# zyang1580/PDA

Measured on AMD Instinct MI355X. Metric: users/sec full-catalogue top-K@50 (eval), higher is better.
Workload: dtype f32; 1 GPU; C3: synthetic 1000000 users x 200000 items, d=128, PDA condition ((elu+1)*pop^0.22) head, masked top-K@50; ranks_seen=1

## Files before the change

pda_amd/csrc/pda_score_topk_v4.hip:

```cpp
#include "pda_v4_shared.h"
#include <cstdlib>
#include <type_traits>

using namespace pda_topk;

namespace {

constexpr int kCap4 = 57;
constexpr int kRing4 = 128;
constexpr int kWarmTiles = 4;
constexpr int kMainWaves = 8;
#ifndef PDA_W4_ABL
#define PDA_W4_ABL 0
#endif
#ifdef PDA_V4_PROF
__device__ unsigned long long pda_prof4[24];
#define PROF_T0(v) const long long v = __builtin_readcyclecounter()
#define PROF_T1(v, slot) prof[slot] += (unsigned long long)(__builtin_readcyclecounter() - v)
#define PROF_INC(slot, x) prof[slot] += (unsigned long long)(x)
#define PROF_FLUSH(first, last) do { if (lane == 0) for (int pq = (first); pq <= (last); ++pq) atomicAdd(&pda_prof4[pq], prof[pq]); } while (0)
#else
#define PROF_T0(v) do {} while (0)
#define PROF_T1(v, slot) do {} while (0)
#define PROF_INC(slot, x) do {} while (0)
// ... 560 lines not shown
    const int cap_t = (g.warm_sorted || g.handover != nullptr || g.warm_final) ? CAP : K;
    auto emit_row = [&](const int r, const uint32_t t, const int c_t) __attribute__((always_inline)) {
        const int row = (r & 3) + 8 * (r >> 2) + 4 * h;
        const int lrow = wave * 32 + row;
        if (j == 0) predt[lrow] = c_t >= K ? pda_unordf(t) : -INFINITY;
        if (__any(c_t > cap_t)) {
#pragma unroll
            for (int k = 0; k < NHT; ++k) {
                const bool p = ordv[k][r] >= t;
                const uint64_t key = ((uint64_t)ordv[k][r] << 32) | (uint64_t)(0xFFFFFFFFu - (uint32_t)itemv[k]);
                append_keys<CAP>(p, lrow, pda_unordf(ordv[k][r]), key, lists, cntl, taul, wave * 32, 32, K, lane);
            }
        } else {
            int run = 0;
#pragma unroll
            for (int k = 0; k < NHT; ++k) {
                const bool p = ordv[k][r] >= t;
                const uint64_t bm = __ballot(p);
                const uint32_t bh = h ? (uint32_t)(bm >> 32) : (uint32_t)bm;
                const int slot = run + __popc(bh & ((1u << j) - 1u));
                if (p) lists[(size_t)lrow * CAP + slot] = ((uint64_t)ordv[k][r] << 32) | (uint64_t)(0xFFFFFFFFu - (uint32_t)itemv[k]);
                run += __popc(bh);
            }
            if (j == 0) cntl[lrow] = run;
        }
    };
#pragma unroll
    for (int r = 0; r < 16; r += 2) {
        if constexpr ((PDA_W4_ABL & 2) != 0) {
#if defined(__HIP_DEVICE_COMPILE__)
#pragma unroll
            for (int k = 0; k < NHT; ++k) asm volatile("" ::"v"(ordv[k][r]), "v"(ordv[k][r + 1]));
#endif
            continue;
        }
        auto count_ge2 = [&](uint32_t ca, uint32_t cb, int& na, int& nb) __attribute__((always_inline)) {
            int loa = 0, hia = 0, lob = 0, hib = 0;
#pragma unroll
            for (int k = 0; k < NHT; ++k) {
                const uint64_t bma = __ballot(ordv[k][r] >= ca);
                const uint64_t bmb = __ballot(ordv[k][r + 1] >= cb);
                loa += __popc((uint32_t)bma);
                hia += __popc((uint32_t)(bma >> 32));
                lob += __popc((uint32_t)bmb);
                hib += __popc((uint32_t)(bmb >> 32));
            }
            na = h ? hia : loa;
            nb = h ? hib : lob;
        };
        int ca_t, cb_t;
        count_ge2(1u, 1u, ca_t, cb_t);
        uint32_t ta = 1u, tb = 1u;
        const bool needa = ca_t > cap_t, needb = cb_t > cap_t;
        if (__any(needa || needb)) {
            uint32_t mxa = 0u, mna = 0xFFFFFFFFu, mxb = 0u, mnb = 0xFFFFFFFFu;
#pragma unroll
            for (int k = 0; k < NHT; ++k) {
                const uint32_t va = ordv[k][r], vb = ordv[k][r + 1];
                mxa = max(mxa, va);
                mna = min(mna, va != 0u ? va : 0xFFFFFFFFu);
                mxb = max(mxb, vb);
                mnb = min(mnb, vb != 0u ? vb : 0xFFFFFFFFu);
            }
#pragma unroll
            for (int o = 16; o >= 1; o >>= 1) {
                mxa = max(mxa, (uint32_t)__shfl_xor((int)mxa, o, 64));
                mna = min(mna, (uint32_t)__shfl_xor((int)mna, o, 64));
                mxb = max(mxb, (uint32_t)__shfl_xor((int)mxb, o, 64));
                mnb = min(mnb, (uint32_t)__shfl_xor((int)mnb, o, 64));
            }
            uint32_t hia = mxa + 1u, hib = mxb + 1u;
            if (needa) ta = mna;
            if (needb) tb = mnb;
            for (int it = 0; it < 40; ++it) {
                const bool opena = needa && ca_t > cap_t && hia - ta > 1u;
                const bool openb = needb && cb_t > cap_t && hib - tb > 1u;
                if (!__any(opena || openb)) break;
                const uint32_t mida = opena ? ta + ((hia - ta) >> 1) : ta;
                const uint32_t midb = openb ? tb + ((hib - tb) >> 1) : tb;
                int cnta, cntb;
                count_ge2(mida, midb, cnta, cntb);
                if (opena) {
                    if (cnta >= K) {
                        ta = mida;
                        ca_t = cnta;
                    } else {
                        hia = mida;
                    }
                }
                if (openb) {
                    if (cntb >= K) {
                        tb = midb;
                        cb_t = cntb;
                    } else {
                        hib = midb;
                    }
                }
            }
        }
        emit_row(r, ta, ca_t);
        emit_row(r + 1, tb, cb_t);
    }
    pda_wave_sync();
    if (tid == 0) atomicAdd(reinterpret_cast<unsigned long long*>(g.stats + 2), (unsigned long long)(2 * nwarm));
    for (int rr = 0; rr < 32; ++rr) {
        uint64_t* buf = my_lists + rr * CAP;
        if (((PDA_W4_ABL & 4) == 0) && (g.warm_sorted || g.warm_final || (g.handover == nullptr && __builtin_amdgcn_readfirstlane(cntl[wave * 32 + rr]) > K)))
            compact_list<CAP>(buf, &cntl[wave * 32 + rr], &taul[wave * 32 + rr], K, lane);
        const int c = cntl[wave * 32 + rr];
        const int rb = utile * kUserTile + wave * 32 + rr;
        if (g.seed_out != nullptr) {
            uint32_t mn = lane < c ? (uint32_t)(buf[lane] >> 32) : 0xFFFFFFFFu;
#pragma unroll
            for (int o = 32; o >= 1; o >>= 1) mn = min(mn, (uint32_t)__shfl_xor((int)mn, o, 64));
            if (lane == 0 && rb < g.n_users_blk) g.seed_out[rb] = c >= K ? pda_unordf(mn) : -INFINITY;
        }
        if (g.kth_ws != nullptr) continue;
        if (g.handover != nullptr) {
            if (rb < g.n_users_blk && lane < CAP) g.handover[((size_t)split * g.n_users_blk + rb) * CAP + lane] = lane < c ? buf[lane] : 0ull;
            if (g.warm_final && rb < g.n_users_blk && lane < K) g.out_keys[((size_t)split * g.n_users_blk + rb) * K + lane] = lane < c ? buf[lane] : 0ull;
        } else if (rb < g.n_users_blk && lane < K) {
            const uint64_t k = lane < c ? buf[lane] : 0ull;
            g.out_keys[((size_t)split * g.n_users_blk + rb) * K + lane] = k;
        }
    }
    if (g.kth_ws != nullptr) {
        pda_wave_sync();
        const int rb0 = utile * kUserTile + wave * 32, nv = max(0, min(32, g.n_users_blk - rb0));
        if (lane < nv) {
            const uint64_t kl = my_lists[(size_t)lane * CAP + (K - 1)];
            g.kth_ws[(size_t)split * g.n_users_blk + rb0 + lane] = cntl[wave * 32 + lane] >= K ? pda_unordf((uint32_t)(kl >> 32)) : -INFINITY;
        }
        uint64_t* ob = g.out_keys + ((size_t)split * g.n_users_blk + rb0) * K;
        const int q64 = 64 / K, r64 = 64 % K;
        int rr = lane / K, p = lane % K;
        for (int i = lane; i < nv * K; i += 64) {
            ob[i] = p < cntl[wave * 32 + rr] ? my_lists[(size_t)rr * CAP + p] : 0ull;
            rr += q64;
            p += r64;
            if (p >= K) { p -= K; ++rr; }
        }
    }
    if (g.pred_ws != nullptr && lane < 32) {
        const int rb = utile * kUserTile + wave * 32 + lane;
        if (rb < g.n_users_blk) {
            g.pred_ws[2 * (size_t)rb] = predt[wave * 32 + lane];
            g.pred_ws[2 * (size_t)rb + 1] = nul[wave * 32 + lane];
        }
    }
}

constexpr int kWS5Waves = 8, kWS5Threads = 64 * kWS5Waves;
constexpr int kWarmPos = 64 * kWarmTiles;
constexpr size_t warm_score5_lds(int d) { return (size_t)kWarmPos * d * 4 + kWarmPos * 8 + (size_t)kWS5Waves * 32 * 2 * kWarmTiles * 4; }

template <int D, bool BF>
__global__ void __launch_bounds__(kWS5Threads) warm_score5_kernel(Args4 g) {
    extern __shared__ __attribute__((aligned(16))) unsigned char smem[];
    constexpr int RB = row_bytes(D);
    constexpr int NC = D / 8;
    constexpr int CPR4 = D / 4;
    float* Bt = reinterpret_cast<float*>(smem);
    float* popw = Bt + kWarmPos * D;
    int* idw = reinterpret_cast<int*>(popw + kWarmPos);
    unsigned* hmask = reinterpret_cast<unsigned*>(idw + kWarmPos);

    const int tid = threadIdx.x, lane = tid & 63, wave = tid >> 6;
    const int j = lane & 31, h = lane >> 5;
    const int nwarm = g.warm_tiles;
    const int npos = 64 * nwarm;
    for (int p = tid; p < npos; p += kWS5Threads) {
        const float* tl = reinterpret_cast<const float*>(g.rows + (size_t)p * RB + 2 * D + 32);
        popw[p] = tl[0];
        idw[p] = reinterpret_cast<const int*>(tl)[1];
    }
    __syncthreads();
    for (int id = tid; id < npos * CPR4; id += kWS5Threads) {
        const int jj = id / CPR4, ch = id % CPR4;
        *reinterpret_cast<f32x4*>(Bt + jj * D + 4 * (ch ^ swz<D>(jj & 31))) = pda_load4<BF>(g.I, (size_t)idw[jj] * D + 4 * ch);
    }
    if (blockIdx.x == 0) {
        for (int p = tid; p < kWarmPos; p += kWS5Threads) g.wscore[p] = p < npos ? (uint32_t)idw[p] : 0u;
        if (tid == 0) g.stats[8] = 5u;
    }
    __syncthreads();

    uint32_t* scores = g.wscore + kWarmPos;
    const int utiles_w = (g.n_users_blk + kUserTile - 1) / kUserTile;
    const int nunits = utiles_w * (kUserTile / 32);
    const int G = (int)gridDim.x, stride = G * kWS5Waves;
    unsigned* hm_l = hmask + wave * 32 * 2 * kWarmTiles;
    static_assert(2 * kWarmTiles == 8, "two 16-byte loads per row");

    auto row_uid = [&](int unit) -> int {
        const int rb = unit * 32 + j;
        return (unit < nunits && rb < g.n_users_blk) ? g.users[rb] : 0;
    };
    auto load_rows = [&](int unit_x, int uid, f32x4 (&a)[NC], u32x4& hm, bool& hm_on) __attribute__((always_inline)) {
        if (unit_x >= nunits) return;
        const int rb = unit_x * 32 + j;
#pragma unroll
        for (int c = 0; c < NC; ++c) a[c] = pda_load4<BF>(g.U, (size_t)uid * D + 4 * h + 8 * c);
        hm_on = false;
        if (g.hmask_tab != nullptr) {
            hm_on = rb < g.n_users_blk && (unsigned)uid < (unsigned)g.hmask_tab_rows;
            hm = *reinterpret_cast<const u32x4*>(g.hmask_tab + (size_t)(hm_on ? uid : 0) * (2 * kWarmTiles) + 4 * h);
        } else if (g.hmask_ws != nullptr) {
            hm_on = true;
            hm = *reinterpret_cast<const u32x4*>(g.hmask_ws + (size_t)rb * (2 * kWarmTiles) + 4 * h);
        }
    };
    unsigned long long n_tiles_done = 0ull;
    auto run_unit = [&](const int unit_in, f32x4 (&areg)[NC], const u32x4& hm_in, const bool hm_on) __attribute__((always_inline)) {
        const int unit = __builtin_amdgcn_readfirstlane(unit_in);
        const int row_blk = unit * 32 + j;
        if (unit * 32 + 32 > g.n_users_blk) {
            const f32x4 z = {0.f, 0.f, 0.f, 0.f};
#pragma unroll
            for (int c = 0; c < NC; ++c) areg[c] = row_blk < g.n_users_blk ? areg[c] : z;
        }
        const u32x4 hz = {0u, 0u, 0u, 0u};
        const u32x4 hmv = hm_on ? hm_in : hz;
        *reinterpret_cast<u32x4*>(hm_l + j * (2 * kWarmTiles) + 4 * h) = hmv;
        {
            constexpr int NK5 = D / 32;
            unsigned char* fb = g.ufrag_out + ((size_t)(row_blk >> 4) * (NK5 * 64) + (size_t)(row_blk & 15)) * 16 + 8 * h;
            float ssc[NC];
#pragma unroll
            for (int c = 0; c < NC; ++c) {
                const f32x4 v = areg[c];
                uint2 w;
                w.x = bf16_rne(v[0]) | (bf16_rne(v[1]) << 16);
                w.y = bf16_rne(v[2]) | (bf16_rne(v[3]) << 16);
                *reinterpret_cast<uint2*>(fb + ((c >> 2) * 64 + 16 * (c & 3)) * 16) = w;
                float ss = 0.f;
#pragma unroll
                for (int k = 0; k < 4; ++k) {
                    const float sq = v[k] * v[k];
                    ss += sq + __shfl_xor(sq, 32, 64);
                }
                ssc[c] = ss;
                __builtin_amdgcn_sched_barrier(0);
            }
#pragma unroll
            for (int o = NC / 2; o > 0; o >>= 1)
#pragma unroll
                for (int c = 0; c < o; ++c) ssc[c] += ssc[c + o];
            if (h == 0) g.unorm_out[row_blk] = sqrtf(ssc[0]) * 1.0009765625f * 1.0001f;
        }
        if ((unit & (kUserTile / 32 - 1)) == 0) n_tiles_done += (unsigned long long)(2 * nwarm);
        pda_wave_sync();
        const int j_lane = j, h_lane = h;
#pragma unroll 1
        for (int ht = 0; ht < 2 * nwarm; ++ht) {
            int j = j_lane, h = h_lane;
#if defined(__HIP_DEVICE_COMPILE__)
            asm volatile("" : "+v"(j), "+v"(h));
#endif
            const int bswz = swz<D>(j);
            const float* brow = Bt + (ht * 32 + j) * D;
            f32x16 acc0 = zero16v(), acc1 = zero16v();
            f32x4 b0 = *reinterpret_cast<const f32x4*>(brow + 4 * (h ^ bswz));
            f32x4 b1 = *reinterpret_cast<const f32x4*>(brow + 4 * ((2 + h) ^ bswz));
#pragma unroll
            for (int c = 0; c < NC; c += 2) {
                f32x4 n0 = b0, n1 = b1;
                if (c + 2 < NC) {
                    n0 = *reinterpret_cast<const f32x4*>(brow + 4 * ((2 * c + 4 + h) ^ bswz));
                    n1 = *reinterpret_cast<const f32x4*>(brow + 4 * ((2 * c + 6 + h) ^ bswz));
                }
#pragma unroll
                for (int q = 0; q < 4; ++q) {
                    acc0 = __builtin_amdgcn_mfma_f32_32x32x2f32(areg[c][q], b0[q], acc0, 0, 0, 0);
                    acc1 = __builtin_amdgcn_mfma_f32_32x32x2f32(areg[c + 1][q], b1[q], acc1, 0, 0, 0);
                }
                __builtin_amdgcn_sched_barrier(0);
                b0 = n0;
                b1 = n1;
            }
            const f32x16 accx = acc0 + acc1;
            const bool okw = (ht * 32 + j) < g.n_items_local;
            const float pv = popw[ht * 32 + j];
            const unsigned hb_mine = hm_l[j * (2 * kWarmTiles) + ht];
            const bool any_hb = __any(hb_mine != 0u);
            const uint32_t soff = (uint32_t)(unit * 32 + 4 * h) * (uint32_t)npos + (uint32_t)(ht * 32 + j);
#pragma unroll
            for (int r = 0; r < 16; ++r) {
                const int row = (r & 3) + 8 * (r >> 2) + 4 * h;
                float sc = accx[r];
                sc = (sc > 0.0f ? sc + 1.0f : __expf(sc)) * pv;
                bool p = okw && (sc >= -INFINITY);
                if (any_hb) {
                    const uint32_t hbr = (uint32_t)__shfl((int)hb_mine, row, 64);
                    if ((hbr >> j) & 1u) p = false;
                }
                scores[soff + (uint32_t)((r & 3) + 8 * (r >> 2)) * (uint32_t)npos] = p ? pda_ordf(sc + 0.0f) : 0u;
            }
        }
        pda_wave_sync();
    };
    int unit = (int)blockIdx.x + G * wave;
    f32x4 ra[NC], rb_[NC];
    u32x4 ha = {0u, 0u, 0u, 0u}, hb = {0u, 0u, 0u, 0u};
    bool oa = false, ob = false;
    load_rows(unit, row_uid(unit), ra, ha, oa);
    int uid_n = row_uid(unit + stride);
    while (unit < nunits) {
        load_rows(unit + stride, uid_n, rb_, hb, ob);
        uid_n = row_uid(unit + 2 * stride);
        run_unit(unit, ra, ha, oa);
        unit += stride;
        if (unit >= nunits) break;
        load_rows(unit + stride, uid_n, ra, ha, oa);
        uid_n = row_uid(unit + 2 * stride);
        run_unit(unit, rb_, hb, ob);
        unit += stride;
    }
    if (lane == 0 && n_tiles_done != 0ull) atomicAdd(reinterpret_cast<unsigned long long*>(g.stats + 2), n_tiles_done);
    if ((int)blockIdx.x == (nunits - 1) % G) {
        const size_t r0 = (size_t)utiles_w * kUserTile, r1 = ((size_t)g.n_users_blk + kUT5 - 1) / kUT5 * kUT5;
        const u32x4 z = {0u, 0u, 0u, 0u};
        for (size_t q = r0 * (2 * D) + (size_t)tid * 16; q < r1 * (2 * D); q += (size_t)kWS5Threads * 16) *reinterpret_cast<u32x4*>(g.ufrag_out + q) = z;
        for (size_t r = r0 + tid; r < r1; r += kWS5Threads) g.unorm_out[r] = 0.f;
    }
}

constexpr int kSelRows = 16;
__global__ void __launch_bounds__(256) __attribute__((amdgpu_waves_per_eu(8))) warm_select5_kernel(Args4 g) {
    constexpr int CAP = kCap4;
    __shared__ uint64_t lists[4][2][64];
    const int tid = threadIdx.x, lane = tid & 63, wave = tid >> 6;
    const int K = g.K, n = g.n_users_blk;
    const int npos = 64 * g.warm_tiles;
    const uint32_t* scores = g.wscore + kWarmPos;
    const int rb0 = ((int)blockIdx.x * 4 + wave) * kSelRows;
    if (rb0 >= n) return;
    const u32x4 idv = *reinterpret_cast<const u32x4*>(g.wscore + 4 * lane);
    uint32_t klo[4];
#pragma unroll
    for (int q = 0; q < 4; ++q) klo[q] = 0xFFFFFFFFu - (uint32_t)(g.item_offset + (int)idv[q]);
    const bool lane_on = 4 * lane < npos;
    float kth_mine = -INFINITY;

    auto count32 = [&](const u32x4& v, uint32_t t) __attribute__((always_inline)) -> int {
        return __popcll(__ballot(v[0] >= t)) + __popcll(__ballot(v[1] >= t)) + __popcll(__ballot(v[2] >= t)) + __popcll(__ballot(v[3] >= t));
    };
    auto key_of = [&](const u32x4& v, int q) __attribute__((always_inline)) -> uint64_t { return ((uint64_t)v[q] << 32) | (uint64_t)klo[q]; };
    auto count64 = [&](const u32x4& v, uint64_t t) __attribute__((always_inline)) -> int {
        int c = 0;
#pragma unroll
        for (int q = 0; q < 4; ++q) c += __popcll(__ballot(key_of(v, q) >= t));
        return c;
    };

#pragma unroll 1
    for (int it = 0; it < kSelRows; it += 2) {
        if (rb0 + it >= n) break;
        u32x4 v[2];
        uint32_t t[2], hi[2];
        int ct[2];
        bool need[2];
#pragma unroll
        for (int s = 0; s < 2; ++s) {
            const int rb = rb0 + it + s;
            const u32x4 z = {0u, 0u, 0u, 0u};
            v[s] = (lane_on && rb < n) ? *reinterpret_cast<const u32x4*>(scores + (size_t)rb * npos + 4 * lane) : z;
        }
#pragma unroll
        for (int s = 0; s < 2; ++s) {
            ct[s] = count32(v[s], 1u);
            t[s] = 1u;
            hi[s] = 0u;
            need[s] = ct[s] > CAP;
        }
        if (need[0] || need[1]) {
#pragma unroll
            for (int s = 0; s < 2; ++s) {
                uint32_t mx = max(max(v[s][0], v[s][1]), max(v[s][2], v[s][3])), mn = 0xFFFFFFFFu;
#pragma unroll
                for (int q = 0; q < 4; ++q) mn = min(mn, v[s][q] != 0u ? v[s][q] : 0xFFFFFFFFu);
#pragma unroll
                for (int o = 32; o >= 1; o >>= 1) {
                    mx = max(mx, (uint32_t)__shfl_xor((int)mx, o, 64));
                    mn = min(mn, (uint32_t)__shfl_xor((int)mn, o, 64));
                }
                hi[s] = (uint32_t)__builtin_amdgcn_readfirstlane((int)mx) + 1u;
                if (need[s]) t[s] = (uint32_t)__builtin_amdgcn_readfirstlane((int)mn);
            }
            for (int step = 0; step < 40; ++step) {
                const bool open0 = need[0] && ct[0] > CAP && hi[0] - t[0] > 1u;
                const bool open1 = need[1] && ct[1] > CAP && hi[1] - t[1] > 1u;
                if (!(open0 || open1)) break;
                const uint32_t mid0 = open0 ? t[0] + ((hi[0] - t[0]) >> 1) : t[0];
                const uint32_t mid1 = open1 ? t[1] + ((hi[1] - t[1]) >> 1) : t[1];
                const int c0 = count32(v[0], mid0), c1 = count32(v[1], mid1);
                if (open0) {
                    if (c0 >= K) { t[0] = mid0; ct[0] = c0; } else { hi[0] = mid0; }
                }
                if (open1) {
                    if (c1 >= K) { t[1] = mid1; ct[1] = c1; } else { hi[1] = mid1; }
                }
            }
        }
        uint64_t thr[2];
#pragma unroll
        for (int s = 0; s < 2; ++s) {
            thr[s] = (uint64_t)t[s] << 32;
            if (ct[s] > CAP) {
                uint64_t lo64 = thr[s], hi64 = (uint64_t)(t[s] + 1u) << 32;
                for (int step = 0; step < 40 && ct[s] > CAP && hi64 - lo64 > 1ull; ++step) {
                    const uint64_t mid = lo64 + ((hi64 - lo64) >> 1);
                    const int c = count64(v[s], mid);
                    if (c >= K) { lo64 = mid; ct[s] = c; } else { hi64 = mid; }
                }
                thr[s] = lo64;
            }
        }
        int cs[2];
#pragma unroll
        for (int s = 0; s < 2; ++s) {
            uint64_t* buf = lists[wave][s];
            int run = 0;
#pragma unroll
            for (int q = 0; q < 4; ++q) {
                const uint64_t key = key_of(v[s], q);
                const bool p = key >= thr[s];
                const uint64_t bm = __ballot(p);
                const int slot = run + (int)__builtin_amdgcn_mbcnt_hi((uint32_t)(bm >> 32), __builtin_amdgcn_mbcnt_lo((uint32_t)bm, 0));
                if (p && slot < 64) buf[slot] = key;
                run += __popcll(bm);
            }
            cs[s] = min(run, CAP);
            if (lane >= cs[s]) buf[lane] = 0ull;
        }
        pda_wave_sync();
        uint64_t key[2];
        int rank[2] = {0, 0};
        key[0] = lists[wave][0][lane];
        key[1] = lists[wave][1][lane];
        const int cm = max(cs[0], cs[1]);
        for (int jj = 0; jj < cm; jj += 4) {
#pragma unroll
            for (int s = 0; s < 2; ++s) {
                const uint64_t* buf = lists[wave][s];
                const uint64_t k0 = buf[jj], k1 = buf[jj + 1], k2 = buf[jj + 2], k3 = buf[jj + 3];
                rank[s] += ((k0 > key[s]) ? 1 : 0) + ((k1 > key[s]) ? 1 : 0) + ((k2 > key[s]) ? 1 : 0) + ((k3 > key[s]) ? 1 : 0);
            }
        }
        pda_wave_sync();
#pragma unroll
        for (int s = 0; s < 2; ++s)
            if (lane < cs[s]) lists[wave][s][rank[s]] = key[s];
        pda_wave_sync();
#pragma unroll
        for (int s = 0; s < 2; ++s) {
            const int rb = rb0 + it + s;
            if (rb < n) {
                if (lane < K) g.out_keys[(size_t)rb * K + lane] = lists[wave][s][lane];
                const uint64_t kl = lists[wave][s][K - 1];
                if (lane == it + s) kth_mine = cs[s] >= K ? pda_unordf((uint32_t)(kl >> 32)) : -INFINITY;
            }
        }
        pda_wave_sync();
    }
    if (lane < kSelRows && rb0 + lane < n) {
        g.kth_ws[rb0 + lane] = kth_mine;
        if (g.seed_out != nullptr) g.seed_out[rb0 + lane] = kth_mine;
    }
}

// ... 1169 lines not shown
        if (phase & 1) g.pred_ws = reinterpret_cast<float*>(g.regroup_ws + 1024 + 2 * (size_t)n_users_blk);
    }

    if (((phase & 1) || from_empty) && hipMemsetAsync(workspace, 0, pda_score_topk_workspace_bytes(n_users_blk), s) != hipSuccess) return PDA_ERR_LAUNCH;
    if (c.bloom) {
        hipLaunchKernelGGL(hist_bloom4_kernel, dim3((unsigned)((n_users_blk + 31) / 32)), dim3(256), 0, s, users, hist_indptr, hist_indices,
                           hist_row_mode, n_users_blk, const_cast<uint32_t*>(g.bloom), g.prep_hdr, pop_head ? 1 : 0);
        PDA_CHECK_LAUNCH();
    }
#define PDA_V4_(DD, BFV) (pop_head ? launch4<DD, PDA_HEAD_POP, BFV>(g, c, s) : launch4<DD, PDA_HEAD_RAW, BFV>(g, c, s))
    switch (d) {
        case 64: return bf16 ? PDA_V4_(64, true) : PDA_V4_(64, false);
        case 128: return bf16 ? PDA_V4_(128, true) : PDA_V4_(128, false);
        case 256: return bf16 ? PDA_V4_(256, true) : PDA_V4_(256, false);
        default: return PDA_ERR_UNSUPPORTED;
    }
#undef PDA_V4_
}

__global__ void __launch_bounds__(256) kth_value_kernel(const uint64_t* __restrict__ keys, int S, int n_users, int K, int pos, float* __restrict__ out) {
    const int u = blockIdx.x * 256 + threadIdx.x;
    if (u >= n_users) return;
    float best = -INFINITY;
    for (int sp = 0; sp < S; ++sp) {
        const uint64_t k = keys[((size_t)sp * n_users + u) * K + pos];
        if (k != 0ull) best = fmaxf(best, pda_key_val(k));
    }
    out[u] = best;
}

__global__ void __launch_bounds__(256) seed_refine_kernel(const uint64_t* __restrict__ keys, int S, int n_users, int K, float* __restrict__ lo,
                                                          float* __restrict__ hi, float* __restrict__ mid, int32_t* __restrict__ counts, int mode) {
    const int u = blockIdx.x * 256 + threadIdx.x;
    if (u >= n_users) return;
    float l = lo[u], h = hi[u];
    if (mode >= 1) {
        if (counts[u] >= K) l = mid[u];
        else h = mid[u];
        lo[u] = l;
        hi[u] = h;
    }
    if (mode <= 1) {
        const bool open = l > -INFINITY && h < INFINITY && h > l;
        const float m = open ? l + 0.5f * (h - l) : l;
        int c = 0;
        for (int sp = 0; sp < S; ++sp) {
            const uint64_t* row = keys + ((size_t)sp * n_users + u) * K;
            for (int q = 0; q < K; ++q) {
                const uint64_t k = row[q];
                if (k == 0ull || pda_key_val(k) < m) break;
                ++c;
            }
        }
        mid[u] = m;
        counts[u] = c;
    }
}


__global__ void __launch_bounds__(256) seed_bounds_kernel(const uint64_t* __restrict__ keys, int S, int n_users, int K, int m,
                                                          float* __restrict__ out) {
    const int u = blockIdx.x * 256 + threadIdx.x;
    if (u >= n_users) return;
    float a = -INFINITY, b = -INFINITY;
    for (int sp = 0; sp < S; ++sp) {
        const uint64_t* row = keys + ((size_t)sp * n_users + u) * K;
        const uint64_t ka = row[K - 1], kb = row[m - 1];
        if (ka != 0ull) a = fmaxf(a, pda_key_val(ka));
        if (kb != 0ull) b = fmaxf(b, pda_key_val(kb));
    }
    out[u] = a;
    out[(size_t)n_users + u] = b;
    out[2 * (size_t)n_users + u] = -b;
}
__device__ __forceinline__ float seed_thr(float lo, float hi, int j, int n_thr) {
    const bool open = lo > -INFINITY && hi < INFINITY && hi > lo;
    return open ? lo + (hi - lo) * ((float)(j + 1) / (float)(n_thr + 1)) : lo;
}
constexpr int kSeedThrMax = 15;
__global__ void __launch_bounds__(256) seed_counts_kernel(const uint64_t* __restrict__ keys, int S, int n_users, int K,
                                                          const float* __restrict__ bounds, int n_thr, int32_t* __restrict__ counts) {
    const int u = blockIdx.x * 256 + threadIdx.x;
    if (u >= n_users) return;
    const float lo = fmaxf(bounds[u], -bounds[2 * (size_t)n_users + u]), hi = bounds[(size_t)n_users + u];
    float thr[kSeedThrMax];
    int c[kSeedThrMax];
#pragma unroll
    for (int j = 0; j < kSeedThrMax; ++j) { thr[j] = seed_thr(lo, hi, j < n_thr ? j : 0, n_thr); c[j] = 0; }
    for (int sp = 0; sp < S; ++sp) {
        const uint64_t* row = keys + ((size_t)sp * n_users + u) * K;
        for (int q = 0; q < K; ++q) {
            const uint64_t k = row[q];
            if (k == 0ull) break;
            const float v = pda_key_val(k);
            if (v < thr[0]) break;
#pragma unroll
            for (int j = 0; j < kSeedThrMax; ++j) c[j] += (v >= thr[j]) ? 1 : 0;
        }
    }
#pragma unroll
    for (int j = 0; j < kSeedThrMax; ++j)
        if (j < n_thr) counts[(size_t)j * n_users + u] = c[j];
}
__global__ void __launch_bounds__(256) seed_pick_kernel(const float* __restrict__ bounds, const int32_t* __restrict__ counts, int n_thr,
                                                        int n_users, int K, float* __restrict__ seed) {
    const int u = blockIdx.x * 256 + threadIdx.x;
    if (u >= n_users) return;
    const float lo = fmaxf(bounds[u], -bounds[2 * (size_t)n_users + u]), hi = bounds[(size_t)n_users + u];
    float s = lo;
    for (int j = 0; j < n_thr; ++j)
        if (counts[(size_t)j * n_users + u] >= K) s = fmaxf(s, seed_thr(lo, hi, j, n_thr));
    seed[u] = s;
}

}

int pda_v4_run_score4_dev(const void* U, const void* I_shard, bool bf16, const void* prep, const float* pop_shard, const int32_t* users, int n_users_blk,
                          const int* n_users_dev, int item_offset, int n_items_local, int d, const int64_t* hist_indptr, const int32_t* hist_indices,
                          int hist_row_mode, int K, int head, int early_stop, int n_splits, const float* seed, uint64_t* out_keys, void* workspace, hipStream_t s) {
    return run_score4(U, I_shard, bf16, prep, pop_shard, users, n_users_blk, item_offset, n_items_local, d, hist_indptr, hist_indices, hist_row_mode, K, head,
                      early_stop, n_splits, out_keys, workspace, s, seed != nullptr ? 4 : 3, seed, 0, n_users_dev);
}

extern "C" int pda_topk_seed_bounds(const uint64_t* keys, int n_splits, int n_users_blk, int K, int m, float* bounds, void* stream) {
    if (!keys || !bounds || n_splits < 1 || n_users_blk < 1 || K < 1 || m < 1 || m > K) return PDA_ERR_ARG;
    hipLaunchKernelGGL(seed_bounds_kernel, dim3((unsigned)((n_users_blk + 255) / 256)), dim3(256), 0, reinterpret_cast<hipStream_t>(stream), keys,
                       n_splits, n_users_blk, K, m, bounds);
    PDA_CHECK_LAUNCH();
    return PDA_OK;
}
extern "C" int pda_topk_seed_counts(const uint64_t* keys, int n_splits, int n_users_blk, int K, const float* bounds, int n_thr, int32_t* counts,
                                    void* stream) {
    if (!keys || !bounds || !counts || n_splits < 1 || n_users_blk < 1 || K < 1 || n_thr < 1 || n_thr > kSeedThrMax) return PDA_ERR_ARG;
    hipLaunchKernelGGL(seed_counts_kernel, dim3((unsigned)((n_users_blk + 255) / 256)), dim3(256), 0, reinterpret_cast<hipStream_t>(stream), keys,
                       n_splits, n_users_blk, K, bounds, n_thr, counts);
    PDA_CHECK_LAUNCH();
    return PDA_OK;
}
extern "C" int pda_topk_seed_pick(const float* bounds, const int32_t* counts, int n_thr, int n_users_blk, int K, float* seed, void* stream) {
    if (!bounds || !seed || n_users_blk < 1 || K < 1 || n_thr < 0 || n_thr > kSeedThrMax || (n_thr > 0 && !counts)) return PDA_ERR_ARG;
    hipLaunchKernelGGL(seed_pick_kernel, dim3((unsigned)((n_users_blk + 255) / 256)), dim3(256), 0, reinterpret_cast<hipStream_t>(stream), bounds,
                       counts, n_thr, n_users_blk, K, seed);
    PDA_CHECK_LAUNCH();
    return PDA_OK;
}

#ifdef PDA_V5_EXITPROF
extern "C" int pda_debug_v5_exitprof(unsigned long long* out, int n_workgroups) {
    if (!out || n_workgroups < 1 || n_workgroups > kXpMaxWg) return PDA_ERR_ARG;
    if (hipMemcpyFromSymbol(out, HIP_SYMBOL(pda_v5_exitprof), (size_t)n_workgroups * 4 * 8 * sizeof(unsigned long long)) != hipSuccess) return PDA_ERR_LAUNCH;
    return PDA_OK;
}
#endif
#ifdef PDA_V4_PROF
extern "C" int pda_debug_prof4(unsigned long long* out16, int reset) {
    if (hipMemcpyFromSymbol(out16, HIP_SYMBOL(pda_prof4), sizeof(unsigned long long) * 24) != hipSuccess) return PDA_ERR_LAUNCH;
    if (reset) { unsigned long long z[24] = {0}; if (hipMemcpyToSymbol(HIP_SYMBOL(pda_prof4), z, sizeof(z)) != hipSuccess) return PDA_ERR_LAUNCH; }
    return PDA_OK;
}
#endif

extern "C" int pda_score_topk4_auto_splits(int n_users_blk, int n_items_local, int d) {
    if (n_users_blk <= 0 || n_items_local <= 0) return 1;
    const int ut = user_tile4(d);
    const int utiles = (n_users_blk + ut - 1) / ut;
    const int n_tiles = (n_items_local + 63) / 64;
    int s = 1;
    while (utiles * s * 2 <= 256 && s < 64 && n_tiles / (s * 2) >= 3 * kWarmTiles) s *= 2;
    return s;
}

extern "C" size_t pda_item_prep4_bytes(int n_items_local, int d) { return n_items_local > 0 ? prep4_layout(n_items_local, d).total : 0; }

extern "C" int pda_item_prep4_f32(const float* I_shard, const float* pop_shard, const int32_t* order, int n_items_local, int d, void* prep,
                                  void* stream) {
    if (!I_shard || !prep || n_items_local <= 0) return PDA_ERR_ARG;
    return run_prep4(I_shard, false, pop_shard, order, n_items_local, d, prep, reinterpret_cast<hipStream_t>(stream));
}
extern "C" int pda_item_prep4_bf16(const uint16_t* I_shard, const float* pop_shard, const int32_t* order, int n_items_local, int d, void* prep,
                                   void* stream) {
    if (!I_shard || !prep || n_items_local <= 0) return PDA_ERR_ARG;
    return run_prep4(I_shard, true, pop_shard, order, n_items_local, d, prep, reinterpret_cast<hipStream_t>(stream));
}
extern "C" int pda_item_prep7_f32(const float* I_shard, const int32_t* order, int n_items_local, int d, void* prep, void* stream) {
    if (!I_shard || !prep || !order || n_items_local <= 0) return PDA_ERR_ARG;
    return run_prep4(I_shard, false, nullptr, order, n_items_local, d, prep, reinterpret_cast<hipStream_t>(stream), 1);
}
extern "C" int pda_item_prep7_bf16(const uint16_t* I_shard, const int32_t* order, int n_items_local, int d, void* prep, void* stream) {
    if (!I_shard || !prep || !order || n_items_local <= 0) return PDA_ERR_ARG;
    return run_prep4(I_shard, true, nullptr, order, n_items_local, d, prep, reinterpret_cast<hipStream_t>(stream), 1);
}
extern "C" int pda_item_prep4_check(const void* prep, int n_items_local, int d, void* stream) {
    if (!prep || n_items_local <= 0) return PDA_ERR_ARG;
    int bad = 0;
    hipStream_t s = reinterpret_cast<hipStream_t>(stream);
    if (hipMemcpyAsync(&bad, prep, 4, hipMemcpyDeviceToHost, s) != hipSuccess) return PDA_ERR_LAUNCH;
    if (hipStreamSynchronize(s) != hipSuccess) return PDA_ERR_LAUNCH;
    return bad ? PDA_ERR_ARG : PDA_OK;
}

extern "C" int pda_topk_kth_value(const uint64_t* keys, int n_splits, int n_users_blk, int K, int pos, float* out, void* stream) {
    if (!keys || !out || n_splits < 1 || n_users_blk < 1 || K < 1 || pos < 0 || pos >= K) return PDA_ERR_ARG;
    hipLaunchKernelGGL(kth_value_kernel, dim3((unsigned)((n_users_blk + 255) / 256)), dim3(256), 0, reinterpret_cast<hipStream_t>(stream), keys,
                       n_splits, n_users_blk, K, pos, out);
    PDA_CHECK_LAUNCH();
    return PDA_OK;
}

extern "C" int pda_topk_seed_refine(const uint64_t* keys, int n_splits, int n_users_blk, int K, float* lo, float* hi, float* mid,
                                    int32_t* counts, int mode, void* stream) {
    if (!keys || !lo || !hi || !mid || !counts || n_splits < 1 || n_users_blk < 1 || K < 1 || mode < 0 || mode > 2) return PDA_ERR_ARG;
    hipLaunchKernelGGL(seed_refine_kernel, dim3((unsigned)((n_users_blk + 255) / 256)), dim3(256), 0, reinterpret_cast<hipStream_t>(stream), keys,
                       n_splits, n_users_blk, K, lo, hi, mid, counts, mode);
    PDA_CHECK_LAUNCH();
    return PDA_OK;
}

extern "C" int pda_score_topk4_phase_f32(const float* U, const float* I_shard, const void* prep, const float* pop_shard, const int32_t* users,
                                         int n_users_blk, int item_offset, int n_items_local, int d, const int64_t* hist_indptr,
                                         const int32_t* hist_indices, int hist_row_mode, int K, int head, int early_stop, int n_splits,
                                         int phase, int warm_tiles, const float* seed, uint64_t* out_keys, void* workspace, void* stream) {
    if (phase != 1 && phase != 2 && phase != 4) return PDA_ERR_ARG;
    return run_score4(U, I_shard, false, prep, pop_shard, users, n_users_blk, item_offset, n_items_local, d, hist_indptr, hist_indices,
                      hist_row_mode, K, head, early_stop, n_splits, out_keys, workspace, reinterpret_cast<hipStream_t>(stream), phase, seed, warm_tiles);
}
extern "C" int pda_score_topk4_phase_bf16(const uint16_t* U, const uint16_t* I_shard, const void* prep, const float* pop_shard,
                                          const int32_t* users, int n_users_blk, int item_offset, int n_items_local, int d,
                                          const int64_t* hist_indptr, const int32_t* hist_indices, int hist_row_mode, int K, int head,
                                          int early_stop, int n_splits, int phase, int warm_tiles, const float* seed, uint64_t* out_keys,
                                          void* workspace, void* stream) {
    if (phase != 1 && phase != 2 && phase != 4) return PDA_ERR_ARG;
    return run_score4(U, I_shard, true, prep, pop_shard, users, n_users_blk, item_offset, n_items_local, d, hist_indptr, hist_indices,
                      hist_row_mode, K, head, early_stop, n_splits, out_keys, workspace, reinterpret_cast<hipStream_t>(stream), phase, seed, warm_tiles);
}

extern "C" int pda_score_topk4_f32(const float* U, const float* I_shard, const void* prep, const float* pop_shard, const int32_t* users,
                                   int n_users_blk, int item_offset, int n_items_local, int d, const int64_t* hist_indptr,
                                   const int32_t* hist_indices, int hist_row_mode, int K, int head, int early_stop, int n_splits,
                                   uint64_t* out_keys, void* workspace, void* stream) {
    return run_score4(U, I_shard, false, prep, pop_shard, users, n_users_blk, item_offset, n_items_local, d, hist_indptr, hist_indices,
                      hist_row_mode, K, head, early_stop, n_splits, out_keys, workspace, reinterpret_cast<hipStream_t>(stream));
}
extern "C" int pda_score_topk4_bf16(const uint16_t* U, const uint16_t* I_shard, const void* prep, const float* pop_shard, const int32_t* users,
                                    int n_users_blk, int item_offset, int n_items_local, int d, const int64_t* hist_indptr,
                                    const int32_t* hist_indices, int hist_row_mode, int K, int head, int early_stop, int n_splits,
                                    uint64_t* out_keys, void* workspace, void* stream) {
    return run_score4(U, I_shard, true, prep, pop_shard, users, n_users_blk, item_offset, n_items_local, d, hist_indptr, hist_indices,
                      hist_row_mode, K, head, early_stop, n_splits, out_keys, workspace, reinterpret_cast<hipStream_t>(stream));
}

extern "C" int pda_score_topk4_phase_masked_f32(const float* U, const float* I_shard, const void* prep, const float* pop_shard, const int32_t* users,
                                                int n_users_blk, int item_offset, int n_items_local, int d, const int64_t* hist_indptr,
                                                const int32_t* hist_indices, int hist_row_mode, int K, int head, int early_stop, int n_splits,
                                                const uint32_t* mask_table, int mask_table_rows, uint64_t* out_keys, void* workspace, void* stream) {
    if (mask_table != nullptr && mask_table_rows <= 0) return PDA_ERR_ARG;
    return run_score4(U, I_shard, false, prep, pop_shard, users, n_users_blk, item_offset, n_items_local, d, hist_indptr, hist_indices,
                      hist_row_mode, K, head, early_stop, n_splits, out_keys, workspace, reinterpret_cast<hipStream_t>(stream), 3, nullptr, 0, nullptr,
                      mask_table, mask_table_rows);
}
extern "C" int pda_score_topk4_phase_masked_bf16(const uint16_t* U, const uint16_t* I_shard, const void* prep, const float* pop_shard, const int32_t* users,
                                                 int n_users_blk, int item_offset, int n_items_local, int d, const int64_t* hist_indptr,
                                                 const int32_t* hist_indices, int hist_row_mode, int K, int head, int early_stop, int n_splits,
                                                 const uint32_t* mask_table, int mask_table_rows, uint64_t* out_keys, void* workspace, void* stream) {
    if (mask_table != nullptr && mask_table_rows <= 0) return PDA_ERR_ARG;
    return run_score4(U, I_shard, true, prep, pop_shard, users, n_users_blk, item_offset, n_items_local, d, hist_indptr, hist_indices,
                      hist_row_mode, K, head, early_stop, n_splits, out_keys, workspace, reinterpret_cast<hipStream_t>(stream), 3, nullptr, 0, nullptr,
                      mask_table, mask_table_rows);
}

static Args4 mask_args4(const void* prep, const int32_t* users, int n_rows, int item_offset, int n_items_local, int d, const int64_t* hist_indptr,
                        const int32_t* hist_indices, int hist_row_mode, int warm_tiles) {
    const Prep4Layout L = prep4_layout(n_items_local, d);
    const unsigned char* pb = reinterpret_cast<const unsigned char*>(prep);
    Args4 g{};
    g.users = users;
    g.hist_indptr = hist_indptr;
    g.hist_indices = hist_indices;
    g.pos_of = reinterpret_cast<const int*>(pb + L.pos_of);
    g.n_users_blk = n_rows;
    g.item_offset = item_offset;
    g.n_items_local = n_items_local;
    g.hist_row_mode = hist_row_mode;
    g.n_splits = 1;
    g.n_tiles = L.n_tiles;
    g.warm_tiles = warm_tiles;
    return g;
}
extern "C" int pda_score_topk4_phase_mask_table(const void* prep, int n_items_local, int d, int item_offset, const int64_t* hist_indptr,
                                                const int32_t* hist_indices, int n_rows, uint32_t* table, void* stream) {
    if (!prep || !hist_indptr || !hist_indices || !table || n_rows <= 0 || n_items_local <= 0 || item_offset < 0) return PDA_ERR_ARG;
    if (d != 64 && d != 128 && d != 256) return PDA_ERR_UNSUPPORTED;
    const Args4 g = mask_args4(prep, nullptr, n_rows, item_offset, n_items_local, d, hist_indptr, hist_indices, PDA_HIST_BY_BLOCK_ROW, kWarmTiles);
    hipLaunchKernelGGL(warm_mask_table4_kernel, dim3((unsigned)((n_rows + kUserTile - 1) / kUserTile)), dim3(kThreads), 0, reinterpret_cast<hipStream_t>(stream), g, table);
    PDA_CHECK_LAUNCH();
    return PDA_OK;
}
extern "C" int pda_score_topk4_phase_mask_rows(const void* prep, const int32_t* users, int n_users_blk, int item_offset, int n_items_local, int d,
                                               const int64_t* hist_indptr, const int32_t* hist_indices, int hist_row_mode, int warm_tiles, uint32_t* out,
                                               void* stream) {
    if (!prep || !users || !hist_indptr || !hist_indices || !out || n_users_blk <= 0 || n_items_local <= 0 || item_offset < 0) return PDA_ERR_ARG;
    if (warm_tiles < 1 || warm_tiles > kWarmTiles) return PDA_ERR_ARG;
    if (d != 64 && d != 128 && d != 256) return PDA_ERR_UNSUPPORTED;
    const Args4 g = mask_args4(prep, users, n_users_blk, item_offset, n_items_local, d, hist_indptr, hist_indices, hist_row_mode, warm_tiles);
    hipLaunchKernelGGL(warm_mask4_kernel, dim3((unsigned)((n_users_blk + kUserTile - 1) / kUserTile)), dim3(kThreads), 0, reinterpret_cast<hipStream_t>(stream), g, out);
    PDA_CHECK_LAUNCH();
    return PDA_OK;
// ... 38 lines not shown
```

Before: 32.76 million users/s.

## Transpose warm-score MFMA output for vectorized score stores and permlane norm reduction

```diff
diff --git a/pda_amd/csrc/pda_score_topk_v4.hip b/pda_amd/csrc/pda_score_topk_v4.hip
--- a/pda_amd/csrc/pda_score_topk_v4.hip
+++ b/pda_amd/csrc/pda_score_topk_v4.hip
@@ -736,6 +736,24 @@
 
 constexpr int kWS5Waves = 8, kWS5Threads = 64 * kWS5Waves;
 constexpr int kWarmPos = 64 * kWarmTiles;
+#ifdef PDA_WS5_PROF
+constexpr int kWs5ProfWg = 256, kWs5ProfUnits = 6, kWs5ProfUnitWords = 1 + 3 * 2 * kWarmTiles, kWs5ProfWords = 4 + kWs5ProfUnits * kWs5ProfUnitWords;
+__device__ unsigned long long pda_ws5_prof[(size_t)kWs5ProfWg * 8 * kWs5ProfWords];
+#define PDA_WS5_STAMP_AT(word)                                                                     \
+    do {                                                                                           \
+        __builtin_amdgcn_sched_barrier(0);                                                         \
+        const unsigned long long t_ = __builtin_amdgcn_s_memtime();                                \
+        if (lane == 0 && prof_w != nullptr) prof_w[word] = t_;                                     \
+        __builtin_amdgcn_sched_barrier(0);                                                         \
+    } while (0)
+#define PDA_WS5_STAMP(slot)                                                                        \
+    do {                                                                                           \
+        if (prof_u < kWs5ProfUnits) PDA_WS5_STAMP_AT(4 + prof_u * kWs5ProfUnitWords + (slot));     \
+    } while (0)
+#else
+#define PDA_WS5_STAMP_AT(word)
+#define PDA_WS5_STAMP(slot)
+#endif
 constexpr size_t warm_score5_lds(int d) { return (size_t)kWarmPos * d * 4 + kWarmPos * 8 + (size_t)kWS5Waves * 32 * 2 * kWarmTiles * 4; }
 
 template <int D, bool BF>
@@ -751,6 +769,11 @@
 
     const int tid = threadIdx.x, lane = tid & 63, wave = tid >> 6;
     const int j = lane & 31, h = lane >> 5;
+#ifdef PDA_WS5_PROF
+    unsigned long long* prof_w = blockIdx.x < (unsigned)kWs5ProfWg ? pda_ws5_prof + ((size_t)blockIdx.x * 8 + wave) * kWs5ProfWords : nullptr;
+    int prof_u = 0;
+#endif
+    PDA_WS5_STAMP_AT(0);
     const int nwarm = g.warm_tiles;
     const int npos = 64 * nwarm;
     for (int p = tid; p < npos; p += kWS5Threads) {
@@ -768,6 +791,7 @@
         if (tid == 0) g.stats[8] = 5u;
     }
     __syncthreads();
+    PDA_WS5_STAMP_AT(1);
 
     uint32_t* scores = g.wscore + kWarmPos;
     const int utiles_w = (g.n_users_blk + kUserTile - 1) / kUserTile;
@@ -797,6 +821,7 @@
     unsigned long long n_tiles_done = 0ull;
     auto run_unit = [&](const int unit_in, f32x4 (&areg)[NC], const u32x4& hm_in, const bool hm_on) __attribute__((always_inline)) {
         const int unit = __builtin_amdgcn_readfirstlane(unit_in);
+        PDA_WS5_STAMP(0);
         const int row_blk = unit * 32 + j;
         if (unit * 32 + 32 > g.n_users_blk) {
             const f32x4 z = {0.f, 0.f, 0.f, 0.f};
@@ -809,25 +834,35 @@
         {
             constexpr int NK5 = D / 32;
             unsigned char* fb = g.ufrag_out + ((size_t)(row_blk >> 4) * (NK5 * 64) + (size_t)(row_blk & 15)) * 16 + 8 * h;
-            float ssc[NC];
-#pragma unroll
-            for (int c = 0; c < NC; ++c) {
-                const f32x4 v = areg[c];
-                uint2 w;
-                w.x = bf16_rne(v[0]) | (bf16_rne(v[1]) << 16);
-                w.y = bf16_rne(v[2]) | (bf16_rne(v[3]) << 16);
-                *reinterpret_cast<uint2*>(fb + ((c >> 2) * 64 + 16 * (c & 3)) * 16) = w;
+            float ssc[NC / 2];
+#pragma unroll
+            for (int c = 0; c < NC / 2; ++c) {
                 float ss = 0.f;
 #pragma unroll
+                for (int e = 0; e < 2; ++e) {
+                    const int ce = c + e * (NC / 2);
+                    const f32x4 v = areg[ce];
+                    uint2 w;
+                    w.x = bf16_rne(v[0]) | (bf16_rne(v[1]) << 16);
+                    w.y = bf16_rne(v[2]) | (bf16_rne(v[3]) << 16);
+                    *reinterpret_cast<uint2*>(fb + ((ce >> 2) * 64 + 16 * (ce & 3)) * 16) = w;
+                }
+                const f32x4 v0 = areg[c], v1 = areg[c + NC / 2];
+#pragma unroll
                 for (int k = 0; k < 4; ++k) {
-                    const float sq = v[k] * v[k];
-                    ss += sq + __shfl_xor(sq, 32, 64);
+                    const auto xy = __builtin_amdgcn_permlane32_swap(__float_as_uint(v0[k] * v0[k]), __float_as_uint(v1[k] * v1[k]), false, false);
+                    ss += __uint_as_float(xy[0]) + __uint_as_float(xy[1]);
                 }
                 ssc[c] = ss;
                 __builtin_amdgcn_sched_barrier(0);
             }
 #pragma unroll
-            for (int o = NC / 2; o > 0; o >>= 1)
+            for (int c = 0; c < NC / 2; ++c) {
+                const auto xy = __builtin_amdgcn_permlane32_swap(__float_as_uint(ssc[c]), __float_as_uint(ssc[c]), false, false);
+                ssc[c] = __uint_as_float(xy[0]) + __uint_as_float(xy[1]);
+            }
+#pragma unroll
+            for (int o = NC / 4; o > 0; o >>= 1)
 #pragma unroll
                 for (int c = 0; c < o; ++c) ssc[c] += ssc[c + o];
             if (h == 0) g.unorm_out[row_blk] = sqrtf(ssc[0]) * 1.0009765625f * 1.0001f;
@@ -841,6 +876,7 @@
 #if defined(__HIP_DEVICE_COMPILE__)
             asm volatile("" : "+v"(j), "+v"(h));
 #endif
+            PDA_WS5_STAMP(1 + 3 * ht);
             const int bswz = swz<D>(j);
             const float* brow = Bt + (ht * 32 + j) * D;
             f32x16 acc0 = zero16v(), acc1 = zero16v();
@@ -855,33 +891,39 @@
                 }
 #pragma unroll
                 for (int q = 0; q < 4; ++q) {
-                    acc0 = __builtin_amdgcn_mfma_f32_32x32x2f32(areg[c][q], b0[q], acc0, 0, 0, 0);
-                    acc1 = __builtin_amdgcn_mfma_f32_32x32x2f32(areg[c + 1][q], b1[q], acc1, 0, 0, 0);
+                    acc0 = __builtin_amdgcn_mfma_f32_32x32x2f32(b0[q], areg[c][q], acc0, 0, 0, 0);
+                    acc1 = __builtin_amdgcn_mfma_f32_32x32x2f32(b1[q], areg[c + 1][q], acc1, 0, 0, 0);
                 }
                 __builtin_amdgcn_sched_barrier(0);
                 b0 = n0;
                 b1 = n1;
             }
             const f32x16 accx = acc0 + acc1;
-            const bool okw = (ht * 32 + j) < g.n_items_local;
-            const float pv = popw[ht * 32 + j];
+            PDA_WS5_STAMP(2 + 3 * ht);
             const unsigned hb_mine = hm_l[j * (2 * kWarmTiles) + ht];
-            const bool any_hb = __any(hb_mine != 0u);
-            const uint32_t soff = (uint32_t)(unit * 32 + 4 * h) * (uint32_t)npos + (uint32_t)(ht * 32 + j);
-#pragma unroll
-            for (int r = 0; r < 16; ++r) {
-                const int row = (r & 3) + 8 * (r >> 2) + 4 * h;
-                float sc = accx[r];
-                sc = (sc > 0.0f ? sc + 1.0f : __expf(sc)) * pv;
-                bool p = okw && (sc >= -INFINITY);
-                if (any_hb) {
-                    const uint32_t hbr = (uint32_t)__shfl((int)hb_mine, row, 64);
-                    if ((hbr >> j) & 1u) p = false;
-                }
-                scores[soff + (uint32_t)((r & 3) + 8 * (r >> 2)) * (uint32_t)npos] = p ? pda_ordf(sc + 0.0f) : 0u;
-            }
+            const uint32_t soff = (uint32_t)(unit * 32 + j) * (uint32_t)npos + (uint32_t)(ht * 32 + 4 * h);
+#pragma unroll
+            for (int gq = 0; gq < 4; ++gq) {
+                const int p0 = ht * 32 + 8 * gq + 4 * h;
+                const f32x4 pv = *reinterpret_cast<const f32x4*>(popw + p0);
+                const unsigned hbg = hb_mine >> (8 * gq + 4 * h);
+                u32x4 o;
+#pragma unroll
+                for (int q = 0; q < 4; ++q) {
+                    float sc = accx[4 * gq + q];
+                    sc = (sc > 0.0f ? sc + 1.0f : __expf(sc)) * pv[q];
+                    bool p = (p0 + q) < g.n_items_local && (sc >= -INFINITY);
+                    if ((hbg >> q) & 1u) p = false;
+                    o[q] = p ? pda_ordf(sc + 0.0f) : 0u;
+                }
+                *reinterpret_cast<u32x4*>(scores + soff + (uint32_t)(8 * gq)) = o;
+            }
+            PDA_WS5_STAMP(3 + 3 * ht);
         }
         pda_wave_sync();
+#ifdef PDA_WS5_PROF
+        ++prof_u;
+#endif
     };
     int unit = (int)blockIdx.x + G * wave;
     f32x4 ra[NC], rb_[NC];
@@ -900,6 +942,10 @@
         run_unit(unit, rb_, hb, ob);
         unit += stride;
     }
+#ifdef PDA_WS5_PROF
+    PDA_WS5_STAMP_AT(2);
+    if (lane == 0 && prof_w != nullptr) prof_w[3] = (unsigned long long)prof_u;
+#endif
     if (lane == 0 && n_tiles_done != 0ull) atomicAdd(reinterpret_cast<unsigned long long*>(g.stats + 2), n_tiles_done);
     if ((int)blockIdx.x == (nunits - 1) % G) {
         const size_t r0 = (size_t)utiles_w * kUserTile, r1 = ((size_t)g.n_users_blk + kUT5 - 1) / kUT5 * kUT5;
@@ -2375,6 +2421,18 @@
     return PDA_OK;
 }
 #endif
+#ifdef PDA_WS5_PROF
+extern "C" int pda_debug_ws5_prof(unsigned long long* out, int n_workgroups) {
+    if (!out || n_workgroups < 1 || n_workgroups > kWs5ProfWg) return PDA_ERR_ARG;
+    if (hipMemcpyFromSymbol(out, HIP_SYMBOL(pda_ws5_prof), (size_t)n_workgroups * 8 * kWs5ProfWords * sizeof(unsigned long long)) != hipSuccess) return PDA_ERR_LAUNCH;
+    return PDA_OK;
+}
+extern "C" int pda_debug_ws5_prof_shape(int* units, int* unit_words, int* words) {
+    if (!units || !unit_words || !words) return PDA_ERR_ARG;
+    *units = kWs5ProfUnits, *unit_words = kWs5ProfUnitWords, *words = kWs5ProfWords;
+    return PDA_OK;
+}
+#endif
 #ifdef PDA_V4_PROF
 extern "C" int pda_debug_prof4(unsigned long long* out16, int reset) {
     if (hipMemcpyFromSymbol(out16, HIP_SYMBOL(pda_prof4), sizeof(unsigned long long) * 24) != hipSuccess) return PDA_ERR_LAUNCH;
```

After: 32.98 million users/s, median of 3. About the same (+0.7%).
